# SeunghwanByun/SemanticSegmentation_Tensorflow

Hardware: AMD Instinct MI355X
Metric: train images/sec on KITTI 375×1242 2-class at 1/2/4/8 MI355X; mIoU parity (higher is better)
Workload: dtype bf16; 1 GPU; FCN (reference Network/model/FCN.py topology) train step: fwd + softmax-xent + bwd + TF1 Adam, 375x1242x3 zero-padded to 384x1248; global_batch=4, batch_per_gpu=4, image=375x1242 -> 384x1248, parallelism=dp1

## Files before the change

semanticsegmentation_tensorflow_amd/csrc/conv.hip:

```cpp
#include "common.h"
#include "igemm.h"
#include "halo.h"
#include <mutex>
#include <stdio.h>
#include <string.h>
#include <math.h>

using seg::NTParams;
using seg::TNParams;

static inline int round8(int c) { return (c + 7) & ~7; }

static int same_pads(int in, int k, int s, int d, int* out, int* pb, int* pa) {
    const int keff = k + (k - 1) * (d - 1);
    *out = (in + s - 1) / s;
    int total = (*out - 1) * s + keff - in;
    if (total < 0) total = 0;
    *pb = total / 2;
    *pa = total - total / 2;
    return 0;
}

static int valid_out(int in, int k, int s, int d) {
    const int keff = k + (k - 1) * (d - 1);
// ... 388 lines not shown
            macs = macs_conv;
            if (op == 1 && bwd_data_strided(d)) {
                if (!bwd_data_strided_ok(d)) return SEG_EINVAL;
                if (bwd_data_s2_runs(d, nullptr)) {
                    fam = "dgrad_s2"; bm = 256; bn = d->C >= 32 ? 32 : 16; sp = 1;
                    break;
                }
                NTParams p = bwd_data_strided_params(d);
                p.epi.n_valid = d->c_valid; p.epi.keep_prob = 1.f;
                fam = seg::nt_choice(p, d->dtype, d->stride_h * d->stride_w, p.M, &bm, &bn, &sp);
                break;
            }
            NTParams p = op == 0 ? conv_fwd_params(d) : conv_bwd_data_params(d);
            p.epi.keep_prob = 1.f;
            if (op == 0 && d->dil_w == d->dil_h && seg::smallc_fwd_ok(p, d->dtype, d->R, d->S, d->dil_h)) {
                fam = "conv_c8"; bm = 512; bn = d->K; sp = 1;
                break;
            }
            fam = seg::nt_choice(p, d->dtype, 1, p.M, &bm, &bn, &sp);
            break;
        }
        case 2: {
            TNParams p = conv_bwd_filter_params(d);
            seg::tn_info(p.M, p.N, p.P, d->dtype, &bm, &bn, &sp);
            fam = "igemm_tn";
            seg::WgradPlan wp;
            if (seg::smallc_wgrad_ok(p, d->dtype)) {
                fam = "wgrad_c8"; bm = 72; bn = p.N; sp = seg::smallc_wgrad_splits(p, seg::device_cus());
            } else if (g_tn_variant == 2 && seg::wgrad_plan(p, d->dtype, seg::device_cus(), &wp)) {
                fam = "wgrad_halo"; bm = 576; bn = wp.nt; sp = wp.splits;
            } else if (g_tn_variant == 2 && seg::tn3_ok(p, d->dtype)) {
                fam = "igemm_tn3"; bm = bn = 256; seg::tn3_info(p.M, p.N, p.P, seg::device_cus(), &sp);
            } else if (g_tn_variant == 2 && d->dtype != SEG_F32 && p.M >= 128) {
                fam = "igemm_tn2";
            }
            macs = macs_conv;
            break;
        }
        case 3: {
            macs = macs_t;
            if (const int kq = tconv_dense_kq(d)) {
                const int M = d->N * d->H * d->W, Nn = d->R * d->S * kq;
                NTParams g = dense_nt(M, Nn, d->C, nullptr, d->ldx, nullptr, nullptr, Nn);
                g.IH = d->H; g.IW = d->W; g.Ha = d->H; g.Wa = d->W; g.OH = d->H; g.OW = d->W;
                fam = seg::nt_choice(g, d->dtype, 1, g.M, &bm, &bn, &sp);
            } else {
                NTParams p = tconv_fwd_params(d);
                fam = seg::nt_choice(p, d->dtype, d->stride_h * d->stride_w, p.M, &bm, &bn, &sp);
            }
            break;
        }
        case 4: {
            macs = macs_t;
            if (const int kq = tconv_dense_kq(d)) {
                const int M = d->N * d->H * d->W, Kd = d->R * d->S * kq;
                NTParams g = dense_nt(M, d->C, Kd, nullptr, Kd, nullptr, nullptr, d->ldx);
                g.IH = d->H; g.IW = d->W; g.Ha = d->H; g.Wa = d->W; g.OH = d->H; g.OW = d->W;
                fam = seg::nt_choice(g, d->dtype, 1, g.M, &bm, &bn, &sp);
            } else {
                NTParams p = tconv_bwd_data_params(d);
                fam = seg::nt_choice(p, d->dtype, 1, p.M, &bm, &bn, &sp);
            }
            break;
        }
        case 5: {
            const int Mt = tconv_dense_kq(d) ? d->R * d->S * tconv_dense_kq(d) : d->R * d->S * d->K;
            seg::tn_info(Mt, d->C, d->N * d->H * d->W, d->dtype, &bm, &bn, &sp);
            fam = (g_tn_variant == 2 && d->dtype != SEG_F32 && Mt >= 128) ? "igemm_tn2" : "igemm_tn";
            if (g_tn_variant == 2 && seg::tn3_applies(Mt, d->C, d->dtype)) {
                fam = "igemm_tn3"; bm = bn = 256; seg::tn3_info(Mt, d->C, d->N * d->H * d->W, seg::device_cus(), &sp);
            }
            macs = macs_t;
            break;
        }
        case 6: {
            NTParams p;
            const int kind = bwd_data_bn_params(d, p);
            if (!kind) return SEG_EINVAL;
            macs = macs_conv;
            if (kind == 1 && seg::bn1x1s_ok(p, d->dtype)) { fam = "bn1x1_stream"; bm = 128; bn = 64; }
            else if (kind == 1) { fam = "igemm_nt2_bn"; bm = 256; bn = 64; }
            else { fam = "conv_res16c_bn"; bm = 256; bn = 64; }
            break;
        }
        case 7: {
            NTParams p = conv_fwd_params(d);
            macs = macs_conv;
            if (seg::s1x1_ok(p, d->dtype, 1)) {
                fam = "conv1x1_stream"; bm = 128; bn = 64;
            } else if (g_nt_variant == 2 && seg::nt2_pro_ok(p, d->dtype, 1)) {
                fam = "igemm_nt2_pro"; bm = 192; bn = p.N <= 64 ? 64 : 128;
            } else {
                fam = "igemm_nt_pro"; bm = 128; bn = p.N <= 64 ? 64 : 128;
            }
            break;
        }
        case 8: {
            TNParams p = conv_bwd_filter_params(d);
            macs = macs_conv;
            seg::tn_info(p.M, p.N, p.P, d->dtype, &bm, &bn, &sp);
            fam = (d->dtype != SEG_F32 && g_tn_variant == 2 && p.M == p.Cg) ? "igemm_tn2_pro" : "igemm_tn_pro";
            break;
        }
        default: return SEG_EINVAL;
    }
    if (name && len > 0) snprintf(name, len, "%s<%s,%d,%d>", fam, ty, bm, bn);
    if (splits) *splits = sp;
    if (flops) *flops = 2.0 * macs;
    return SEG_OK;
}

namespace {
struct Knob {
    const char* name;
    std::atomic<int> seg::KnobSet::*var;
    int lo, hi;
    int step;
    int only[8];
};

std::mutex g_knob_mu;

const Knob* find_knob(const char* name) {
    static const Knob knobs[] = {
        {"igemm_nt_variant", &seg::KnobSet::nt_variant, 1, 2, 1, {}},
        {"igemm_tn_variant", &seg::KnobSet::tn_variant, 1, 2, 1, {}},
        {"tn_nsplit", &seg::KnobSet::tn_nsplit, 0, 1, 1, {}},
        {"nt_nsplit", &seg::KnobSet::nt_nsplit, 0, 1, 1, {}},
        {"halo_duo", &seg::KnobSet::halo_duo, 0, 1, 1, {}},
        {"nt_halo", &seg::KnobSet::nt_halo, 0, 1, 1, {}},
        {"halo_wide", &seg::KnobSet::halo_wide, 0, 1, 1, {}},
        {"halo4", &seg::KnobSet::halo4, 0, 2, 1, {}},
        {"halo_min_splits", &seg::KnobSet::halo_min_splits, 1, 64, 1, {}},
        {"adam_tr_fused", &seg::KnobSet::adam_tr_fused, 0, 1, 1, {}},
        {"nt2_short", &seg::KnobSet::nt2_short, 0, 64, 1, {}},
        {"tn_fill", &seg::KnobSet::tn_fill, 1, 64, 1, {}},
        {"tn_split_cap", &seg::KnobSet::tn_split_cap, 1, 4096, 1, {}},
        {"tn_reduce_sl", &seg::KnobSet::tn_reduce_sl, 0, 0, 0, {1, 2, 4, 8, 16, 32, 64}},
        {"tn2_smallm", &seg::KnobSet::tn2_smallm, 0, 1, 1, {}},
        {"adam_blocks", &seg::KnobSet::adam_blocks, 0, 1 << 30, 1, {}},
        {"nt3_fill", &seg::KnobSet::nt3_fill, 0, 1, 1, {}},
        {"tn3_stagger_us", &seg::KnobSet::tn3_stagger_us, 0, 1000, 1, {}},
        {"s1x1", &seg::KnobSet::s1x1, 0, 1, 1, {}},
        {"tn3_half", &seg::KnobSet::tn3_half, 0, 7, 1, {}},
        {"tn3_mfast", &seg::KnobSet::tn3_mfast, 0, 1, 1, {}},
        {"tn3", &seg::KnobSet::tn3, 0, 1, 1, {}},
        {"nt3", &seg::KnobSet::nt3, 0, 1, 1, {}},
        {"wgrad_fill", &seg::KnobSet::wgrad_fill, 1, 800, 1, {}},
        {"wgrad_nt32", &seg::KnobSet::wgrad_nt32, 0, 1, 1, {}},
        {"wgrad_nbias", &seg::KnobSet::wgrad_nbias, 1, 4, 1, {}},
        {"wgrad_nt", &seg::KnobSet::wgrad_nt, 0, 0, 0, {64, 128}},
        {"wgrad_halo", &seg::KnobSet::wgrad_halo, 0, 1, 1, {}},
        {"wgrad_pxs", &seg::KnobSet::wgrad_pxs, 0, 1, 1, {}},
        {"smallc_tr", &seg::KnobSet::smallc_tr, 0, 1, 1, {}},
        {"res16c", &seg::KnobSet::res16c, 0, 1, 1, {}},
        {"res16", &seg::KnobSet::res16, 0, 1, 1, {}},
        {"res64", &seg::KnobSet::res64, 0, 1, 1, {}},
        {"res64_pp", &seg::KnobSet::res64_pp, 0, 2, 1, {}},
        {"res16_dma", &seg::KnobSet::res16_dma, 0, 1, 1, {}},
        {"res16c_bh", &seg::KnobSet::res16c_bh, 0, 0, 0, {4, 8}},
        {"bn1x1s", &seg::KnobSet::bn1x1s, 0, 1, 1, {}},
        {"s1x1_st", &seg::KnobSet::s1x1_st, 0, 2, 1, {}},
        {"res16c_st", &seg::KnobSet::res16c_st, 0, 1, 1, {}},
        {"dropout_flat", &seg::KnobSet::dropout_flat, 0, 1, 1, {}},
        {"smallc", &seg::KnobSet::smallc, 0, 1, 1, {}},
        {"smallk", &seg::KnobSet::smallk, 0, 1, 1, {}},
        {"wpad", &seg::KnobSet::wpad, 0, 256, 8, {}},
        {"dgrad_s2", &seg::KnobSet::dgrad_s2, 0, 1, 1, {}},
#ifdef SEG_DIAG
        {"tn3_abl", &seg::KnobSet::tn3_abl, 0, 3, 1, {}},
        {"smallk_abl", &seg::KnobSet::smallk_abl, 0, 3, 1, {}},
        {"tn3_adam_abl", &seg::KnobSet::tn3_adam_abl, 0, 31, 1, {}},
        {"wgrad_abl", &seg::KnobSet::wgrad_abl, 0, 3, 1, {}},
        {"nt2_ablate", &seg::KnobSet::nt2_ablate, 0, 19, 1, {}},
        {"res64_abl", &seg::KnobSet::res64_abl, 0, 5, 1, {}},
#endif
    };
    for (const Knob& k : knobs)
        if (!strcmp(name, k.name)) return &k;
    return nullptr;
}
}

namespace seg {
KnobSet& knobs() {
    constexpr int MAXDEV = 64;
    static KnobSet sets[MAXDEV];
    int d = 0;
    if (hipGetDevice(&d) != hipSuccess || d < 0 || d >= MAXDEV) d = 0;
    return sets[d];
}
}

extern "C" int seg_set_option(const char* name, int value) {
    const Knob* k = name ? find_knob(name) : nullptr;
    if (!k) return SEG_EINVAL;
    bool ok;
    if (k->step) {
        ok = value >= k->lo && value <= k->hi && (value - k->lo) % k->step == 0;
    } else {
        ok = false;
        for (int v : k->only) ok = ok || (v != 0 && v == value);
    }
    if (!ok) return SEG_EINVAL;
    std::lock_guard<std::mutex> lk(g_knob_mu);
    (seg::knobs().*(k->var)).store(value, std::memory_order_relaxed);
    return SEG_OK;
}

extern "C" int seg_get_option(const char* name, int* value) {
    const Knob* k = name ? find_knob(name) : nullptr;
    if (!k || !value) return SEG_EINVAL;
    *value = (seg::knobs().*(k->var)).load(std::memory_order_relaxed);
    return SEG_OK;
}

extern "C" int seg_conv2d_fwd(const seg_conv_desc* d, const void* x, const void* w, const seg_epilogue* epi,
                              void* y, void* ws, size_t ws_bytes, void* stream) {
    int st = check_desc(d);
    if (st) return st;
    if (!x || !w || !y) return SEG_EINVAL;
    NTParams p = conv_fwd_params(d);
    p.x = x; p.w = w; p.y = y;
    p.epi = make_epi(epi, d->k_valid, (long)d->OH * d->OW * (epi ? epi->ld_residual : 0));
    if (d->dil_w == d->dil_h && seg::smallc_fwd_ok(p, d->dtype, d->R, d->S, d->dil_h)) {
        seg::launch_smallc_fwd(p, d->dtype, (hipStream_t)stream);
        SEG_CHECK_LAUNCH();
        return SEG_OK;
    }
    return seg::launch_nt(p, d->dtype, 1, p.M, ws, ws_bytes, (hipStream_t)stream);
}

static bool fwd_relu_bits_params(const seg_conv_desc* d, const seg_epilogue* epi, int ld_bits, NTParams* out) {
    if (check_desc(d) || d->dil_w != d->dil_h || ld_bits < d->K / 8 || (d->K == 64 && ld_bits % 8)) return false;
    if (epi && epi->relu_mask) return false;
    NTParams p = conv_fwd_params(d);
    p.epi = make_epi(epi, d->k_valid, (long)d->OH * d->OW * (epi ? epi->ld_residual : 0));
    if (!seg::smallc_fwd_ok(p, d->dtype, d->R, d->S, d->dil_h)) return false;
    p.epi.ld_bits = ld_bits;
    *out = p;
    return true;
}

extern "C" int seg_conv2d_fwd_relu_bits_ok(const seg_conv_desc* d) {
    NTParams p;
    seg_epilogue e = {};
    e.relu = 1;
    e.keep_prob = 1.f;
    return d && fwd_relu_bits_params(d, &e, d->K / 8, &p) ? 1 : 0;
}

extern "C" int seg_conv2d_fwd_relu_bits(const seg_conv_desc* d, const void* x, const void* w, const seg_epilogue* epi,
                                        void* y, void* bits, int ld_bits, void* stream) {
    if (!d || !x || !w || !y || !bits) return SEG_EINVAL;
    if (d->K == 64 && ((uintptr_t)bits & 7)) return SEG_EALIGN;
    NTParams p;
    if (!fwd_relu_bits_params(d, epi, ld_bits, &p)) return SEG_EINVAL;
    p.x = x; p.w = w; p.y = y;
    p.epi.ybits = reinterpret_cast<unsigned char*>(bits);
    seg::launch_smallc_fwd(p, d->dtype, (hipStream_t)stream);
    SEG_CHECK_LAUNCH();
    return SEG_OK;
}

static NTParams fwd_hwio_params(const seg_conv_desc* d) {
    NTParams p = conv_fwd_params(d);
    p.bt = 1;
    p.w_col = d->K + g_wpad;
    p.w_tap = (long)d->C * (d->K + g_wpad);
    return p;
}

extern "C" int seg_conv2d_fwd_hwio_ok(const seg_conv_desc* d) {
    if (!d || check_desc(d) || (d->dtype != SEG_BF16 && d->dtype != SEG_F16)) return 0;
    return seg::nt_fwd_bt_ok(fwd_hwio_params(d), d->dtype) ? 1 : 0;
}

extern "C" int seg_conv2d_fwd_hwio(const seg_conv_desc* d, const void* x, const void* w_hwio, const seg_epilogue* epi,
                                   void* y, void* ws, size_t ws_bytes, void* stream) {
    int st = check_desc(d);
    if (st) return st;
    if (!x || !w_hwio || !y) return SEG_EINVAL;
    if (!seg_conv2d_fwd_hwio_ok(d)) return SEG_EINVAL;
    NTParams p = fwd_hwio_params(d);
    p.x = x; p.w = w_hwio; p.y = y;
    p.epi = make_epi(epi, d->k_valid, (long)d->OH * d->OW * (epi ? epi->ld_residual : 0));
    return seg::launch_nt(p, d->dtype, 1, p.M, ws, ws_bytes, (hipStream_t)stream);
}

static bool fwd_pool_params(const seg_conv_desc* d, const seg_epilogue* epi, NTParams* out) {
    if (check_desc(d) || (d->dtype != SEG_BF16 && d->dtype != SEG_F16)) return false;
    if ((d->OH & 1) || (d->OW & 1) || d->OH < 2 || d->OW < 2) return false;
    if (epi && (epi->scale || epi->shift || epi->residual || epi->relu_mask || (epi->keep_prob > 0.f && epi->keep_prob < 1.f)))
        return false;
    NTParams p = conv_fwd_params(d);
    p.epi = make_epi(epi, d->k_valid, 0);
    if (d->dil_w == d->dil_h && seg::smallc_fwd_ok(p, d->dtype, d->R, d->S, d->dil_h)) return false;
    if (!seg::nt_pool_ok(p, d->dtype)) return false;
    *out = p;
    return true;
}

extern "C" int seg_conv2d_fwd_pool_ok(const seg_conv_desc* d) {
    if (!d) return 0;
    NTParams p;
    seg_epilogue e = {};
// ... 635 lines not shown
```

semanticsegmentation_tensorflow_amd/csrc/knobs.h:

```cpp
#pragma once
#include <atomic>

namespace seg {

#define SEG_KNOBS(X) \
    X(wpad, 0) \
    X(adam_tr_fused, 0) \
    X(s1x1, 1) \
    X(bn1x1s, 1) \
    X(s1x1_st, 1) \
    X(dropout_flat, 1) \
    X(nt_halo, 1) \
    X(halo_wide, 1) \
    X(res64, 1) \
    X(res16, 1) \
    X(res64_pp, 1) \
    X(res64_abl, 0) \
    X(wgrad_pxs, 1) \
    X(smallc_tr, 1) \
    X(res16_dma, 1) \
    X(res16c_bh, 4) \
    X(res16c, 1) \
    X(halo_duo, 1) \
    X(halo_min_splits, 1) \
    X(res16c_st, 1) \
    X(halo4, 2) \
    X(nt_nsplit, 1) \
    X(tn_nsplit, 1) \
    X(nt_variant, 2) \
    X(nt3_fill, 1) \
    X(tn_variant, 2) \
    X(tn_fill, 2) \
    X(tn_split_cap, 256) \
    X(tn2_smallm, 0) \
    X(tn_reduce_sl, 16) \
    X(nt2_ablate, 0) \
    X(nt2_short, 8) \
    X(nt3, 1) \
    X(tn3, 1) \
    X(tn3_abl, 0) \
    X(tn3_mfast, 0) \
    X(tn3_half, 0) \
    X(tn3_stagger_us, 40) \
    X(tn3_adam_abl, 0) \
    X(adam_blocks, 0) \
    X(smallc, 1) \
    X(smallk, 1) \
    X(smallk_abl, 0) \
    X(wgrad_halo, 1) \
    X(wgrad_nt, 128) \
    X(wgrad_abl, 0) \
    X(wgrad_nt32, 1) \
    X(wgrad_fill, 88) \
    X(wgrad_nbias, 1) \
    X(dgrad_s2, 1)

struct KnobSet {
#define SEG_KNOB_MEMBER(n, d) std::atomic<int> n{d};
    SEG_KNOBS(SEG_KNOB_MEMBER)
#undef SEG_KNOB_MEMBER
};

KnobSet& knobs();

}

#define g_wpad (::seg::knobs().wpad.load(std::memory_order_relaxed))
#define g_adam_tr_fused (::seg::knobs().adam_tr_fused.load(std::memory_order_relaxed))
#define g_s1x1 (::seg::knobs().s1x1.load(std::memory_order_relaxed))
#define g_bn1x1s (::seg::knobs().bn1x1s.load(std::memory_order_relaxed))
#define g_s1x1_st (::seg::knobs().s1x1_st.load(std::memory_order_relaxed))
#define g_dropout_flat (::seg::knobs().dropout_flat.load(std::memory_order_relaxed))
#define g_nt_halo (::seg::knobs().nt_halo.load(std::memory_order_relaxed))
#define g_halo_wide (::seg::knobs().halo_wide.load(std::memory_order_relaxed))
#define g_res64 (::seg::knobs().res64.load(std::memory_order_relaxed))
#define g_res16 (::seg::knobs().res16.load(std::memory_order_relaxed))
#define g_res64_pp (::seg::knobs().res64_pp.load(std::memory_order_relaxed))
#define g_res64_abl (::seg::knobs().res64_abl.load(std::memory_order_relaxed))
#define g_wgrad_pxs (::seg::knobs().wgrad_pxs.load(std::memory_order_relaxed))
#define g_smallc_tr (::seg::knobs().smallc_tr.load(std::memory_order_relaxed))
#define g_res16_dma (::seg::knobs().res16_dma.load(std::memory_order_relaxed))
#define g_res16c_bh (::seg::knobs().res16c_bh.load(std::memory_order_relaxed))
#define g_res16c (::seg::knobs().res16c.load(std::memory_order_relaxed))
#define g_halo_duo (::seg::knobs().halo_duo.load(std::memory_order_relaxed))
#define g_halo_min_splits (::seg::knobs().halo_min_splits.load(std::memory_order_relaxed))
#define g_res16c_st (::seg::knobs().res16c_st.load(std::memory_order_relaxed))
#define g_halo4 (::seg::knobs().halo4.load(std::memory_order_relaxed))
#define g_nt_nsplit (::seg::knobs().nt_nsplit.load(std::memory_order_relaxed))
#define g_tn_nsplit (::seg::knobs().tn_nsplit.load(std::memory_order_relaxed))
#define g_nt_variant (::seg::knobs().nt_variant.load(std::memory_order_relaxed))
#define g_nt3_fill (::seg::knobs().nt3_fill.load(std::memory_order_relaxed))
#define g_tn_variant (::seg::knobs().tn_variant.load(std::memory_order_relaxed))
#define g_tn_fill (::seg::knobs().tn_fill.load(std::memory_order_relaxed))
#define g_tn_split_cap (::seg::knobs().tn_split_cap.load(std::memory_order_relaxed))
#define g_tn2_smallm (::seg::knobs().tn2_smallm.load(std::memory_order_relaxed))
#define g_tn_reduce_sl (::seg::knobs().tn_reduce_sl.load(std::memory_order_relaxed))
#define g_nt2_ablate (::seg::knobs().nt2_ablate.load(std::memory_order_relaxed))
#define g_nt2_short (::seg::knobs().nt2_short.load(std::memory_order_relaxed))
#define g_nt3 (::seg::knobs().nt3.load(std::memory_order_relaxed))
#define g_tn3 (::seg::knobs().tn3.load(std::memory_order_relaxed))
#define g_tn3_abl (::seg::knobs().tn3_abl.load(std::memory_order_relaxed))
#define g_tn3_mfast (::seg::knobs().tn3_mfast.load(std::memory_order_relaxed))
#define g_tn3_half (::seg::knobs().tn3_half.load(std::memory_order_relaxed))
#define g_tn3_stagger_us (::seg::knobs().tn3_stagger_us.load(std::memory_order_relaxed))
#define g_tn3_adam_abl (::seg::knobs().tn3_adam_abl.load(std::memory_order_relaxed))
#define g_adam_blocks (::seg::knobs().adam_blocks.load(std::memory_order_relaxed))
#define g_smallc (::seg::knobs().smallc.load(std::memory_order_relaxed))
#define g_smallk (::seg::knobs().smallk.load(std::memory_order_relaxed))
#define g_smallk_abl (::seg::knobs().smallk_abl.load(std::memory_order_relaxed))
#define g_wgrad_halo (::seg::knobs().wgrad_halo.load(std::memory_order_relaxed))
#define g_wgrad_nt (::seg::knobs().wgrad_nt.load(std::memory_order_relaxed))
#define g_wgrad_abl (::seg::knobs().wgrad_abl.load(std::memory_order_relaxed))
#define g_wgrad_nt32 (::seg::knobs().wgrad_nt32.load(std::memory_order_relaxed))
#define g_wgrad_fill (::seg::knobs().wgrad_fill.load(std::memory_order_relaxed))
#define g_wgrad_nbias (::seg::knobs().wgrad_nbias.load(std::memory_order_relaxed))
#define g_dgrad_s2 (::seg::knobs().dgrad_s2.load(std::memory_order_relaxed))
```

semanticsegmentation_tensorflow_amd/csrc/wgrad.hip:

```cpp
#include "common.h"
#include "igemm.h"
#include "ldsdma.h"

namespace seg {

static __device__ uint4 wg_zero_page[4];


struct WGGeom {
    int tiles_x, tiles_y, nimg, hwd, hrows;
    int nct, nnt, splits, tps, ptiles;
    int nbias;
};

template <int ROWB>
__device__ __forceinline__ int wg_swz(int row) {
    if constexpr (ROWB >= 256) return ((row & 3) << 1) | (((row >> 3) & 1) << 3);
    else if constexpr (ROWB == 64) return 0;
    else return (((row >> 1) & 1) << 1) | (((row >> 3) & 1) << 2);
}

template <int NT, int NST, int HI, int ABL = 0, typename T = bf16, bool PXS = false>
__global__ __launch_bounds__(512) void wgrad_halo(TNParams p, WGGeom g) {
    constexpr int BW = 16;
    using V8 = vec8_t<T>;
    constexpr int NW = 8, BH = 128 / BW;
    constexpr int NF = PXS ? NT / 16 : NT / 32;
    static_assert(!PXS || NT == 64, "pixel-split waves hold all 64 columns");
    constexpr int DROWB = NT * 2;
    constexpr int D_RPI = 1024 / DROWB;
    constexpr int D_INS = 128 / D_RPI / NW;
    constexpr int D_CPR = DROWB / 16;
    constexpr int HBUF = HI * NW * 1024;
    constexpr int DBUF = 128 * DROWB;
    constexpr int STAGE = HBUF + DBUF;
    static_assert(BW == 16 || BW == 32, "8-pixel fragment groups must stay in one tile row");
    __shared__ __attribute__((aligned(16))) char smem[NST * STAGE];

    const int nout = g.nct * g.nnt;
    const int wg = xcd_remap2(blockIdx.x, gridDim.x);
    const int split = wg / nout, ot = wg - (wg / nout) * nout;
    if (split >= g.splits) return;
    const int ct = ot / g.nnt, nt = ot - (ot / g.nnt) * g.nnt;
    const int c0 = ct * 64, n0 = nt * NT;
    const int t_begin = split * g.tps, t_end = min(g.ptiles, t_begin + g.tps);

    const int tid = threadIdx.x, lane = tid & 63;
    const int w = __builtin_amdgcn_readfirstlane(tid >> 6);
    const int cf = w & 3;
    const int nh = PXS ? 0 : w >> 2;
    const int ph = PXS ? w >> 2 : 0;
    const T* __restrict__ X = reinterpret_cast<const T*>(p.x);
    const T* __restrict__ Dy = reinterpret_cast<const T*>(p.b);
    const void* zero = (const void*)wg_zero_page;

    const int lr = lane >> 3;
    const int hc = (lane & 7) ^ ((((lr >> 1) & 1) << 1) | ((w & 1) << 2));
    int h_hy[HI], h_hx[HI];
#pragma unroll
    for (int h = 0; h < HI; ++h) {
        const int hr = (h * NW + w) * 8 + lr;
        h_hy[h] = hr < g.hrows ? hr / g.hwd : -(1 << 20);
        h_hx[h] = hr < g.hrows ? hr - (hr / g.hwd) * g.hwd : 0;
    }
    const int h_n = g.hrows > w * 8 ? min(HI, (g.hrows - w * 8 + NW * 8 - 1) / (NW * 8)) : 0;
    const int dr = lane / D_CPR, dpc = lane % D_CPR;
    int dc;
    if constexpr (DROWB >= 256) dc = dpc ^ (((dr & 3) << 1) | (((w >> 1) & 1) << 3));
    else if constexpr (DROWB == 64) dc = dpc;
    else dc = dpc ^ ((((dr >> 1) & 1) << 1) | ((w & 1) << 2));
    const bool d_nok = n0 + dc * 8 < p.N;

    const unsigned lds0 = (unsigned)(uintptr_t)(SEG_LDS char*)smem;
    auto stage_tile = [&](int t, int buf) {
        const int tpi = g.tiles_x * g.tiles_y;
        const int img = t / tpi;
        const int rem = t - img * tpi;
        const int ty = rem / g.tiles_x, tx = rem - (rem / g.tiles_x) * g.tiles_x;
        const int oy0 = ty * BH, ox0 = tx * BW;
        const long xb = (long)img * p.x_img + c0 + hc * 8;
        const unsigned sb = lds0 + buf * STAGE;
#pragma unroll
        for (int h = 0; h < HI; ++h) {
            if (h < h_n) {
                const int ih = oy0 + p.ioh + h_hy[h], iw = ox0 + p.iow + h_hx[h];
                const bool ok = (unsigned)ih < (unsigned)p.IH && (unsigned)iw < (unsigned)p.IW;
                const void* src = ok ? (const void*)(X + xb + ((long)ih * p.IW + iw) * p.ldx) : zero;
                glds16(src, sb + (h * NW + w) * 1024);
            }
        }
#pragma unroll
        for (int i = 0; i < D_INS; ++i) {
            const int r = (i * NW + w) * D_RPI + dr;
            const int oy = oy0 + r / BW, ox = ox0 + r % BW;
            const bool ok = d_nok && oy < p.Ha && ox < p.Wa;
            const void* src =
                ok ? (const void*)(Dy + (((long)img * p.Ha + oy) * p.Wa + ox) * p.ldb + n0 + dc * 8) : zero;
            glds16(src, sb + HBUF + (i * NW + w) * 1024);
        }
    };

    f32x4 acc[9][NF];
#pragma unroll
    for (int i = 0; i < 9; ++i)
#pragma unroll
        for (int j = 0; j < NF; ++j) acc[i][j] = f32x4{0.f, 0.f, 0.f, 0.f};
    const bool do_bias = p.dbias != nullptr && ct < g.nbias && cf < NF;
    float dsum[NF];
#pragma unroll
    for (int j = 0; j < NF; ++j) dsum[j] = 0.f;

    const int fg = lane >> 4, tq = (lane & 15) >> 2, tpp = lane & 3;
    typedef short s16x8 __attribute__((ext_vector_type(8)));
    int tapoff[9];
#pragma unroll
    for (int r = 0; r < 3; ++r)
#pragma unroll
        for (int s = 0; s < 3; ++s) tapoff[r * 3 + s] = r * p.tsh * g.hwd + s * p.tsw;

    unsigned a_pk[9], b_pk[NF];
    {
        const int kk = 8 * fg + tq;
        const int py = kk / BW, px = kk - (kk / BW) * BW;
        const int achk = cf * 2 + (tpp >> 1);
#pragma unroll
        for (int t = 0; t < 9; ++t) {
            const int r1 = py * g.hwd + px + tapoff[t];
            const unsigned lo = r1 * 128 + 16 * (achk ^ wg_swz<128>(r1)) + 8 * (tpp & 1);
            const unsigned hi = (r1 + 4) * 128 + 16 * (achk ^ wg_swz<128>(r1 + 4)) + 8 * (tpp & 1);
            a_pk[t] = lo | (hi << 16);
        }
        const int d1 = wg_swz<DROWB>(kk), d2 = wg_swz<DROWB>(kk + 4);
#pragma unroll
        for (int ni = 0; ni < NF; ++ni) {
            const int chk = ((nh * (NT / 2) + ni * 16) >> 3) + (tpp >> 1);
            const unsigned lo = kk * DROWB + 16 * ((chk & ~15) | ((chk & 15) ^ d1)) + 8 * (tpp & 1);
            const unsigned hi = (kk + 4) * DROWB + 16 * ((chk & ~15) | ((chk & 15) ^ d2)) + 8 * (tpp & 1);
            b_pk[ni] = lo | (hi << 16);
        }
    }
    const int per_tile = h_n + D_INS;
    for (int i = 0; i < NST - 1; ++i)
        if (t_begin + i < t_end) stage_tile(t_begin + i, i);
    int buf = 0;
    for (int t = t_begin; t < t_end; ++t) {
        const int younger = min(NST - 2, t_end - 1 - t);
        const int allow = younger * per_tile;
        if (allow <= 0) wait_vmcnt<0>();
        else if (allow <= 2) wait_vmcnt<2>();
        else if (allow <= 3) wait_vmcnt<3>();
        else if (allow <= 4) wait_vmcnt<4>();
        else if (allow <= 5) wait_vmcnt<5>();
        else if (allow <= 6) wait_vmcnt<6>();
        else if (allow <= 7) wait_vmcnt<7>();
        else if (allow <= 8) wait_vmcnt<8>();
        else if (allow <= 9) wait_vmcnt<9>();
        else if (allow <= 10) wait_vmcnt<10>();
        else if (allow <= 11) wait_vmcnt<11>();
        else wait_vmcnt<12>();
        lds_barrier();
        if (ABL != 1 && t + NST - 1 < t_end) stage_tile(t + NST - 1, buf == 0 ? NST - 1 : buf - 1);
        auto read_b = [&](int ss, V8* bo) {
            if constexpr (ABL == 3) {
#pragma unroll
                for (int ni = 0; ni < NF; ++ni) {
                    s16x8 v = {(short)ss, (short)ni, 1, 2, 3, 4, 5, (short)lane};
                    bo[ni] = __builtin_bit_cast(V8, v);
                }
                return;
            }
#pragma unroll
            for (int ni = 0; ni < NF; ++ni) {
                SEG_LDS char* dbs = (SEG_LDS char*)smem + buf * STAGE + HBUF + ss * 32 * DROWB;
                const s16x4 lo = __builtin_amdgcn_ds_read_tr16_b64_v4i16((SEG_LDS s16x4*)(dbs + (b_pk[ni] & 0xffffu)));
                const s16x4 hi = __builtin_amdgcn_ds_read_tr16_b64_v4i16((SEG_LDS s16x4*)(dbs + (b_pk[ni] >> 16)));
                s16x8 v = {lo[0], lo[1], lo[2], lo[3], hi[0], hi[1], hi[2], hi[3]};
                bo[ni] = __builtin_bit_cast(V8, v);
                if (do_bias && ni == cf && ss % g.nbias == ct) {
#pragma unroll
                    for (int e = 0; e < 8; ++e)
                        dsum[ni] += bits16_to_f32<T>((unsigned short)v[e]);
                }
            }
        };
        auto read_a = [&](int ss, int tap) {
            if constexpr (ABL == 3) {
                s16x8 v = {(short)ss, (short)tap, 1, 2, 3, 4, 5, (short)lane};
                return __builtin_bit_cast(V8, v);
            }
            SEG_LDS char* hb = (SEG_LDS char*)smem + buf * STAGE + ss * (32 / BW) * g.hwd * 128;
            const s16x4 lo = __builtin_amdgcn_ds_read_tr16_b64_v4i16((SEG_LDS s16x4*)(hb + (a_pk[tap] & 0xffffu)));
            const s16x4 hi = __builtin_amdgcn_ds_read_tr16_b64_v4i16((SEG_LDS s16x4*)(hb + (a_pk[tap] >> 16)));
            s16x8 v = {lo[0], lo[1], lo[2], lo[3], hi[0], hi[1], hi[2], hi[3]};
            return __builtin_bit_cast(V8, v);
        };
        const int ss0 = 2 * ph;
        V8 b0[NF], b1[NF];
        read_b(ss0, b0);
        V8 a_cur = read_a(ss0, 0);
        auto substep = [&](int ss, V8* bc, V8* bn, bool more) {
#pragma unroll
            for (int tap = 0; tap < 9; ++tap) {
                V8 a_nxt = a_cur;
                if (tap < 8) a_nxt = read_a(ss, tap + 1);
                else if (more) a_nxt = read_a(ss + 1, 0);
                if (tap == 4 && more) read_b(ss + 1, bn);
#pragma unroll
                for (int ni = 0; ni < NF; ++ni) {
                    if constexpr (ABL == 2) asm volatile("" ::"v"(a_cur), "v"(bc[ni]));
                    else acc[tap][ni] = mfma_v8<T>(a_cur, bc[ni], acc[tap][ni]);
                }
                a_cur = a_nxt;
            }
        };
        if constexpr (PXS) {
            substep(ss0, b0, b1, true);
            substep(ss0 + 1, b1, b0, false);
        } else {
#pragma unroll 1
            for (int ss = 0; ss < 4; ss += 2) {
                substep(ss, b0, b1, true);
                substep(ss + 1, b1, b0, ss + 2 < 4);
            }
        }
        buf = buf == NST - 1 ? 0 : buf + 1;
    }
    const int fr = lane & 15;
    const int slab = PXS ? 2 * split + ph : split;
    if (do_bias) {
#pragma unroll
        for (int ni = 0; ni < NF; ++ni) {
            dsum[ni] += __shfl_xor(dsum[ni], 16);
            dsum[ni] += __shfl_xor(dsum[ni], 32);
        }
        if (fg == 0) {
#pragma unroll
            for (int ni = 0; ni < NF; ++ni) {
                if (ni != cf) continue;
                const int n = n0 + nh * (NT / 2) + ni * 16 + fr;
                if (p.partial) {
                    if (n < p.N) p.partial[((long)slab * p.Mp + p.M + ct) * p.N + n] = dsum[ni];
                } else if (n < p.n_valid) {
                    p.dbias[n] = dsum[ni];
                }
            }
        }
    }
#pragma unroll
    for (int tap = 0; tap < 9; ++tap)
#pragma unroll
        for (int j = 0; j < 4; ++j) {
            const int c = c0 + cf * 16 + fg * 4 + j;
            const int m = tap * p.Cg + c;
            if (p.partial) {
                float* prow = p.partial + ((long)slab * p.Mp + m) * p.N;
#pragma unroll
                for (int ni = 0; ni < NF; ++ni) {
                    const int n = n0 + nh * (NT / 2) + ni * 16 + fr;
                    if (n < p.N) prow[n] = acc[tap][ni][j];
                }
            } else if (c < p.c_valid) {
                float* orow = p.out + (long)tap * p.o_tap + (long)c * p.o_c;
#pragma unroll
                for (int ni = 0; ni < NF; ++ni) {
                    const int n = n0 + nh * (NT / 2) + ni * 16 + fr;
                    if (n < p.n_valid) orow[(long)n * p.o_n] = acc[tap][ni][j];
                }
            }
        }
}

bool wgrad_plan(const TNParams& p, int dtype, int cus, WgradPlan* wp) {
    if (!g_wgrad_halo || (dtype != SEG_BF16 && dtype != SEG_F16)) return false;
    if (p.ish != 1 || p.isw != 1 || p.taps_w != 3 || p.Cg % 64 != 0 || p.M != 9 * p.Cg) return false;
    if (p.tsh <= 0 || p.tsw <= 0 || p.N % 8 != 0 || p.ldb % 8 != 0 || p.ldx % 8 != 0) return false;
    if (p.Ha <= 0 || p.Wa <= 0 || p.P % (p.Ha * p.Wa) != 0) return false;
    const int nimg = p.P / (p.Ha * p.Wa);
    const int bw = 16, bh = 128 / bw;
    const int hwd = (bw + 2 * p.tsw + 7) & ~7;
    const int hrows = hwd * (bh + 2 * p.tsh);
    if (hrows > 5 * 64) return false;
    wp->bw = bw;
    wp->g[0] = (p.Wa + bw - 1) / bw; wp->g[1] = (p.Ha + bh - 1) / bh; wp->g[3] = hwd; wp->g[4] = hrows;
    wp->nt = (g_wgrad_nt == 128 && p.N > 64 && wp->g[4] <= 4 * 64) ? 128 : 64;
    if (g_wgrad_nt32 && p.N <= 32) wp->nt = 32;
    wp->g[2] = nimg;
    const int nct = p.Cg / 64, nnt = (p.N + wp->nt - 1) / wp->nt;
    const int nout = nct * nnt;
    const int ptiles = nimg * wp->g[0] * wp->g[1];
    const int tcus = std::max(1, cus * g_wgrad_fill / 100);
    int splits = std::max(1, std::min(ptiles, one_round_splits(nout, tcus, ptiles)));
    const int tps = (ptiles + splits - 1) / splits;
    splits = (ptiles + tps - 1) / tps;
    wp->g[5] = nct; wp->g[6] = nnt; wp->g[7] = splits; wp->g[8] = tps; wp->g[9] = ptiles;
    wp->splits = splits;
    wp->pxs = wp->nt == 64 && g_wgrad_pxs && splits > 1;
    wp->slabs = splits * (wp->pxs ? 2 : 1);
    wp->nbias = splits > 1 ? std::max(1, std::min(nct, g_wgrad_nbias)) : 1;
    wp->blocks = (long)nout * splits;
    return true;
}

size_t wgrad_workspace(const WgradPlan& wp, const TNParams& p) {
    return wp.slabs > 1 ? (size_t)wp.slabs * (p.M + wp.nbias) * p.N * sizeof(float) : 0;
}

void launch_wgrad(TNParams& p, const WgradPlan& wp, hipStream_t s, int dtype) {
    WGGeom g;
    g.tiles_x = wp.g[0]; g.tiles_y = wp.g[1]; g.nimg = wp.g[2]; g.hwd = wp.g[3]; g.hrows = wp.g[4];
    g.nct = wp.g[5]; g.nnt = wp.g[6]; g.splits = wp.g[7]; g.tps = wp.g[8]; g.ptiles = wp.g[9];
    g.nbias = wp.nbias;
    const dim3 grid((unsigned)wp.blocks), block(512);
    const bool small = g.hrows <= 4 * 64;
#ifdef SEG_DIAG
    if (g_wgrad_abl && wp.nt == 128 && dtype == SEG_BF16) {
        if (g_wgrad_abl == 1) hipLaunchKernelGGL((wgrad_halo<128, 2, 4, 1>), grid, block, 0, s, p, g);
        if (g_wgrad_abl == 2) hipLaunchKernelGGL((wgrad_halo<128, 2, 4, 2>), grid, block, 0, s, p, g);
        if (g_wgrad_abl == 3) hipLaunchKernelGGL((wgrad_halo<128, 2, 4, 3>), grid, block, 0, s, p, g);
        return;
    }
#endif
    if (wp.pxs) {
        if (dtype == SEG_F16) {
            if (small) hipLaunchKernelGGL((wgrad_halo<64, 3, 4, 0, f16, true>), grid, block, 0, s, p, g);
            else hipLaunchKernelGGL((wgrad_halo<64, 2, 5, 0, f16, true>), grid, block, 0, s, p, g);
        } else {
            if (small) hipLaunchKernelGGL((wgrad_halo<64, 3, 4, 0, bf16, true>), grid, block, 0, s, p, g);
            else hipLaunchKernelGGL((wgrad_halo<64, 2, 5, 0, bf16, true>), grid, block, 0, s, p, g);
        }
        return;
    }
    if (dtype == SEG_F16) {
        if (wp.nt == 128) hipLaunchKernelGGL((wgrad_halo<128, 2, 4, 0, f16>), grid, block, 0, s, p, g);
        else if (wp.nt == 32 && small) hipLaunchKernelGGL((wgrad_halo<32, 3, 4, 0, f16>), grid, block, 0, s, p, g);
        else if (wp.nt == 32) hipLaunchKernelGGL((wgrad_halo<32, 2, 5, 0, f16>), grid, block, 0, s, p, g);
        else if (small) hipLaunchKernelGGL((wgrad_halo<64, 3, 4, 0, f16>), grid, block, 0, s, p, g);
        else hipLaunchKernelGGL((wgrad_halo<64, 2, 5, 0, f16>), grid, block, 0, s, p, g);
        return;
    }
    if (wp.nt == 128) hipLaunchKernelGGL((wgrad_halo<128, 2, 4>), grid, block, 0, s, p, g);
    else if (wp.nt == 32 && small) hipLaunchKernelGGL((wgrad_halo<32, 3, 4>), grid, block, 0, s, p, g);
    else if (wp.nt == 32) hipLaunchKernelGGL((wgrad_halo<32, 2, 5>), grid, block, 0, s, p, g);
    else if (small) hipLaunchKernelGGL((wgrad_halo<64, 3, 4>), grid, block, 0, s, p, g);
    else hipLaunchKernelGGL((wgrad_halo<64, 2, 5>), grid, block, 0, s, p, g);
}

}
```

Measured before the change: 609.9 images/s.

## Interleave wgrad halo tile staging loads between MFMA groups

Adds an SB variant of the wgrad_halo kernel. It precomputes buffer resource descriptors and per-piece offsets, then issues the next tile's global-to-LDS loads one piece at a time after every second MFMA tap, rather than in a single burst before compute. Tile and image indices are advanced incrementally instead of being recomputed with divisions. The goal is to hide load issue and address arithmetic behind matrix math. In exchange it uses more registers, and it is gated by a 31-bit range check on buffer sizes.

```diff
diff --git a/semanticsegmentation_tensorflow_amd/csrc/conv.hip b/semanticsegmentation_tensorflow_amd/csrc/conv.hip
--- a/semanticsegmentation_tensorflow_amd/csrc/conv.hip
+++ b/semanticsegmentation_tensorflow_amd/csrc/conv.hip
@@ -564,6 +564,7 @@
         {"wgrad_nt", &seg::KnobSet::wgrad_nt, 0, 0, 0, {64, 128}},
         {"wgrad_halo", &seg::KnobSet::wgrad_halo, 0, 1, 1, {}},
         {"wgrad_pxs", &seg::KnobSet::wgrad_pxs, 0, 1, 1, {}},
+        {"wgrad_stage", &seg::KnobSet::wgrad_stage, 0, 1, 1, {}},
         {"smallc_tr", &seg::KnobSet::smallc_tr, 0, 1, 1, {}},
         {"res16c", &seg::KnobSet::res16c, 0, 1, 1, {}},
         {"res16", &seg::KnobSet::res16, 0, 1, 1, {}},
diff --git a/semanticsegmentation_tensorflow_amd/csrc/knobs.h b/semanticsegmentation_tensorflow_amd/csrc/knobs.h
--- a/semanticsegmentation_tensorflow_amd/csrc/knobs.h
+++ b/semanticsegmentation_tensorflow_amd/csrc/knobs.h
@@ -53,6 +53,7 @@
     X(wgrad_nt32, 1) \
     X(wgrad_fill, 88) \
     X(wgrad_nbias, 1) \
+    X(wgrad_stage, 1) \
     X(dgrad_s2, 1)
 
 struct KnobSet {
@@ -114,4 +115,5 @@
 #define g_wgrad_nt32 (::seg::knobs().wgrad_nt32.load(std::memory_order_relaxed))
 #define g_wgrad_fill (::seg::knobs().wgrad_fill.load(std::memory_order_relaxed))
 #define g_wgrad_nbias (::seg::knobs().wgrad_nbias.load(std::memory_order_relaxed))
+#define g_wgrad_stage (::seg::knobs().wgrad_stage.load(std::memory_order_relaxed))
 #define g_dgrad_s2 (::seg::knobs().dgrad_s2.load(std::memory_order_relaxed))
diff --git a/semanticsegmentation_tensorflow_amd/csrc/wgrad.hip b/semanticsegmentation_tensorflow_amd/csrc/wgrad.hip
--- a/semanticsegmentation_tensorflow_amd/csrc/wgrad.hip
+++ b/semanticsegmentation_tensorflow_amd/csrc/wgrad.hip
@@ -20,7 +20,7 @@
     else return (((row >> 1) & 1) << 1) | (((row >> 3) & 1) << 2);
 }
 
-template <int NT, int NST, int HI, int ABL = 0, typename T = bf16, bool PXS = false>
+template <int NT, int NST, int HI, int ABL = 0, typename T = bf16, bool PXS = false, bool SB = false>
 __global__ __launch_bounds__(512) void wgrad_halo(TNParams p, WGGeom g) {
     constexpr int BW = 16;
     using V8 = vec8_t<T>;
@@ -72,6 +72,84 @@
     const bool d_nok = n0 + dc * 8 < p.N;
 
     const unsigned lds0 = (unsigned)(uintptr_t)(SEG_LDS char*)smem;
+
+    constexpr unsigned OOB = 0x80000000u;
+    constexpr int NPIECE = HI + D_INS;
+    const unsigned hv0 = (unsigned)((lr * p.ldx + hc * 8) * 2);
+    const unsigned dv0 = d_nok ? (unsigned)((dr * p.ldb + dc * 8) * 2) : OOB;
+    int p_hy[HI], p_hx[HI];
+    unsigned p_off[HI];
+#pragma unroll
+    for (int h = 0; h < HI; ++h) {
+        const int hr0 = (h * NW + w) * 8;
+        p_hy[h] = hr0 / g.hwd;
+        p_hx[h] = hr0 - p_hy[h] * g.hwd;
+        p_off[h] = (unsigned)((p_hy[h] * p.IW + p_hx[h]) * p.ldx * 2);
+    }
+    int s_tx = 0, s_ty = 0;
+    unsigned s_xoff = 0, s_doff = 0;
+    const T* s_xb = X;
+    const T* s_db = Dy;
+    seg_i32x4 rs_x = {0, 0, 0, 0x00020000}, rs_d = {0, 0, 0, 0x00020000};
+    auto s_set_img = [&]() {
+        const uint64_t xa = (uint64_t)(uintptr_t)s_xb, da = (uint64_t)(uintptr_t)s_db;
+        rs_x.x = (int)(unsigned)xa; rs_x.y = (int)((xa >> 32) & 0xffffu);
+        rs_d.x = (int)(unsigned)da; rs_d.y = (int)((da >> 32) & 0xffffu);
+    };
+    auto s_set_tile = [&]() {
+        s_xoff = (unsigned)((((s_ty * BH) * p.IW + s_tx * BW) * p.ldx + c0) * 2);
+        s_doff = (unsigned)((((s_ty * BH) * p.Wa + s_tx * BW) * p.ldb + n0) * 2);
+    };
+    auto s_advance = [&]() {
+        if (++s_tx == g.tiles_x) {
+            s_tx = 0;
+            if (++s_ty == g.tiles_y) {
+                s_ty = 0;
+                s_xb += p.x_img;
+                s_db += (long)p.Ha * p.Wa * p.ldb;
+                s_set_img();
+            }
+        }
+        s_set_tile();
+    };
+    if constexpr (SB) {
+        const int tpi = g.tiles_x * g.tiles_y;
+        const int img = t_begin / tpi;
+        const int rem = t_begin - img * tpi;
+        s_ty = rem / g.tiles_x;
+        s_tx = rem - s_ty * g.tiles_x;
+        const int shift = (p.ioh * p.IW + p.iow) * p.ldx;
+        s_xb = X + (long)img * p.x_img + shift;
+        s_db = Dy + (long)img * p.Ha * p.Wa * p.ldb;
+        rs_x.z = (p.IH * p.IW * p.ldx - shift) * 2;
+        rs_d.z = p.Ha * p.Wa * p.ldb * 2;
+        s_set_img();
+        s_set_tile();
+    }
+    auto s_piece = [&](const int K, unsigned sb) __attribute__((always_inline)) {
+        if (K < HI) {
+            if (K < h_n) {
+                const bool rok = (unsigned)(s_ty * BH + p.ioh + p_hy[K]) < (unsigned)p.IH;
+                const bool cok = (unsigned)(s_tx * BW + p.iow + p_hx[K] + lr) < (unsigned)p.IW;
+                bglds16(rs_x, rok && cok ? hv0 : OOB, rok ? s_xoff + p_off[K] : 0u, sb + (K * NW + w) * 1024);
+            }
+        } else if (K < NPIECE) {
+            const int I = K - HI;
+            const int rr = (I * NW + w) * D_RPI;
+            const int oyo = rr / BW, oxo = rr % BW;
+            const bool rok = s_ty * BH + oyo < p.Ha;
+            const bool cok = s_tx * BW + oxo + dr < p.Wa;
+            bglds16(rs_d, rok && cok ? dv0 : OOB, rok ? s_doff + (unsigned)((oyo * p.Wa + oxo) * p.ldb * 2) : 0u,
+                    sb + HBUF + (I * NW + w) * 1024);
+        }
+    };
+    auto s_burst = [&](unsigned sb) {
+#pragma unroll
+        for (int k = 0; k < NPIECE; ++k) s_piece(k, sb);
+        s_advance();
+    };
+    static_assert(NPIECE <= 9, "one piece after every second MFMA group of two substeps");
+
     auto stage_tile = [&](int t, int buf) {
         const int tpi = g.tiles_x * g.tiles_y;
         const int img = t / tpi;
@@ -141,7 +219,10 @@
     }
     const int per_tile = h_n + D_INS;
     for (int i = 0; i < NST - 1; ++i)
-        if (t_begin + i < t_end) stage_tile(t_begin + i, i);
+        if (t_begin + i < t_end) {
+            if constexpr (SB) s_burst(lds0 + i * STAGE);
+            else stage_tile(t_begin + i, i);
+        }
     int buf = 0;
     for (int t = t_begin; t < t_end; ++t) {
         const int younger = min(NST - 2, t_end - 1 - t);
@@ -159,7 +240,11 @@
         else if (allow <= 11) wait_vmcnt<11>();
         else wait_vmcnt<12>();
         lds_barrier();
-        if (ABL != 1 && t + NST - 1 < t_end) stage_tile(t + NST - 1, buf == 0 ? NST - 1 : buf - 1);
+        const bool st_on = ABL != 1 && t + NST - 1 < t_end;
+        const unsigned st_sb = lds0 + (buf == 0 ? NST - 1 : buf - 1) * STAGE;
+        if constexpr (!SB) {
+            if (st_on) stage_tile(t + NST - 1, buf == 0 ? NST - 1 : buf - 1);
+        }
         auto read_b = [&](int ss, V8* bo) {
             if constexpr (ABL == 3) {
 #pragma unroll
@@ -198,7 +283,8 @@
         V8 b0[NF], b1[NF];
         read_b(ss0, b0);
         V8 a_cur = read_a(ss0, 0);
-        auto substep = [&](int ss, V8* bc, V8* bn, bool more) {
+        auto substep = [&](int ss, V8* bc, V8* bn, bool more, bool st, auto sec_tag) __attribute__((always_inline)) {
+            constexpr int G0 = decltype(sec_tag)::value ? 9 : 0;
 #pragma unroll
             for (int tap = 0; tap < 9; ++tap) {
                 V8 a_nxt = a_cur;
@@ -211,16 +297,28 @@
                     else acc[tap][ni] = mfma_v8<T>(a_cur, bc[ni], acc[tap][ni]);
                 }
                 a_cur = a_nxt;
+                if constexpr (SB) {
+                    if ((G0 + tap) % 2 == 0 && (G0 + tap) / 2 < NPIECE) {
+                        if (st) s_piece((G0 + tap) / 2, st_sb);
+                    }
+                }
             }
         };
         if constexpr (PXS) {
-            substep(ss0, b0, b1, true);
-            substep(ss0 + 1, b1, b0, false);
+            substep(ss0, b0, b1, true, st_on, std::false_type{});
+            substep(ss0 + 1, b1, b0, false, st_on, std::true_type{});
+            if constexpr (SB) {
+                if (st_on) s_advance();
+            }
         } else {
 #pragma unroll 1
             for (int ss = 0; ss < 4; ss += 2) {
-                substep(ss, b0, b1, true);
-                substep(ss + 1, b1, b0, ss + 2 < 4);
+                const bool st = st_on && ss == 0;
+                substep(ss, b0, b1, true, st, std::false_type{});
+                substep(ss + 1, b1, b0, ss + 2 < 4, st, std::true_type{});
+                if constexpr (SB) {
+                    if (st) s_advance();
+                }
             }
         }
         buf = buf == NST - 1 ? 0 : buf + 1;
@@ -305,44 +403,58 @@
     return wp.slabs > 1 ? (size_t)wp.slabs * (p.M + wp.nbias) * p.N * sizeof(float) : 0;
 }
 
+static bool wgrad_stage_ok(const TNParams& p) {
+    const long shift = ((long)p.ioh * p.IW + p.iow) * p.ldx;
+    const long xb = ((long)(p.IH + 32) * p.IW * p.ldx + std::labs(shift)) * 2;
+    const long db = (long)(p.Ha + 32) * p.Wa * p.ldb * 2;
+    return (long)p.IH * p.IW * p.ldx - shift > 0 && xb < (1L << 31) && db < (1L << 31);
+}
+
+template <int NT, int NST, int HI, int ABL, typename T, bool PXS>
+static void wgrad_launch1(bool sb, dim3 grid, hipStream_t s, const TNParams& p, const WGGeom& g) {
+    if (sb) hipLaunchKernelGGL((wgrad_halo<NT, NST, HI, ABL, T, PXS, true>), grid, dim3(512), 0, s, p, g);
+    else hipLaunchKernelGGL((wgrad_halo<NT, NST, HI, ABL, T, PXS, false>), grid, dim3(512), 0, s, p, g);
+}
+
 void launch_wgrad(TNParams& p, const WgradPlan& wp, hipStream_t s, int dtype) {
     WGGeom g;
     g.tiles_x = wp.g[0]; g.tiles_y = wp.g[1]; g.nimg = wp.g[2]; g.hwd = wp.g[3]; g.hrows = wp.g[4];
     g.nct = wp.g[5]; g.nnt = wp.g[6]; g.splits = wp.g[7]; g.tps = wp.g[8]; g.ptiles = wp.g[9];
     g.nbias = wp.nbias;
-    const dim3 grid((unsigned)wp.blocks), block(512);
+    const dim3 grid((unsigned)wp.blocks);
     const bool small = g.hrows <= 4 * 64;
+    const bool sb = g_wgrad_stage && wgrad_stage_ok(p);
 #ifdef SEG_DIAG
     if (g_wgrad_abl && wp.nt == 128 && dtype == SEG_BF16) {
-        if (g_wgrad_abl == 1) hipLaunchKernelGGL((wgrad_halo<128, 2, 4, 1>), grid, block, 0, s, p, g);
-        if (g_wgrad_abl == 2) hipLaunchKernelGGL((wgrad_halo<128, 2, 4, 2>), grid, block, 0, s, p, g);
-        if (g_wgrad_abl == 3) hipLaunchKernelGGL((wgrad_halo<128, 2, 4, 3>), grid, block, 0, s, p, g);
+        if (g_wgrad_abl == 1) wgrad_launch1<128, 2, 4, 1, bf16, false>(sb, grid, s, p, g);
+        if (g_wgrad_abl == 2) wgrad_launch1<128, 2, 4, 2, bf16, false>(sb, grid, s, p, g);
+        if (g_wgrad_abl == 3) wgrad_launch1<128, 2, 4, 3, bf16, false>(sb, grid, s, p, g);
         return;
     }
 #endif
     if (wp.pxs) {
         if (dtype == SEG_F16) {
-            if (small) hipLaunchKernelGGL((wgrad_halo<64, 3, 4, 0, f16, true>), grid, block, 0, s, p, g);
-            else hipLaunchKernelGGL((wgrad_halo<64, 2, 5, 0, f16, true>), grid, block, 0, s, p, g);
+            if (small) wgrad_launch1<64, 3, 4, 0, f16, true>(sb, grid, s, p, g);
+            else wgrad_launch1<64, 2, 5, 0, f16, true>(sb, grid, s, p, g);
         } else {
-            if (small) hipLaunchKernelGGL((wgrad_halo<64, 3, 4, 0, bf16, true>), grid, block, 0, s, p, g);
-            else hipLaunchKernelGGL((wgrad_halo<64, 2, 5, 0, bf16, true>), grid, block, 0, s, p, g);
+            if (small) wgrad_launch1<64, 3, 4, 0, bf16, true>(sb, grid, s, p, g);
+            else wgrad_launch1<64, 2, 5, 0, bf16, true>(sb, grid, s, p, g);
         }
         return;
     }
     if (dtype == SEG_F16) {
-        if (wp.nt == 128) hipLaunchKernelGGL((wgrad_halo<128, 2, 4, 0, f16>), grid, block, 0, s, p, g);
-        else if (wp.nt == 32 && small) hipLaunchKernelGGL((wgrad_halo<32, 3, 4, 0, f16>), grid, block, 0, s, p, g);
-        else if (wp.nt == 32) hipLaunchKernelGGL((wgrad_halo<32, 2, 5, 0, f16>), grid, block, 0, s, p, g);
-        else if (small) hipLaunchKernelGGL((wgrad_halo<64, 3, 4, 0, f16>), grid, block, 0, s, p, g);
-        else hipLaunchKernelGGL((wgrad_halo<64, 2, 5, 0, f16>), grid, block, 0, s, p, g);
+        if (wp.nt == 128) wgrad_launch1<128, 2, 4, 0, f16, false>(sb, grid, s, p, g);
+        else if (wp.nt == 32 && small) wgrad_launch1<32, 3, 4, 0, f16, false>(sb, grid, s, p, g);
+        else if (wp.nt == 32) wgrad_launch1<32, 2, 5, 0, f16, false>(sb, grid, s, p, g);
+        else if (small) wgrad_launch1<64, 3, 4, 0, f16, false>(sb, grid, s, p, g);
+        else wgrad_launch1<64, 2, 5, 0, f16, false>(sb, grid, s, p, g);
         return;
     }
-    if (wp.nt == 128) hipLaunchKernelGGL((wgrad_halo<128, 2, 4>), grid, block, 0, s, p, g);
-    else if (wp.nt == 32 && small) hipLaunchKernelGGL((wgrad_halo<32, 3, 4>), grid, block, 0, s, p, g);
-    else if (wp.nt == 32) hipLaunchKernelGGL((wgrad_halo<32, 2, 5>), grid, block, 0, s, p, g);
-    else if (small) hipLaunchKernelGGL((wgrad_halo<64, 3, 4>), grid, block, 0, s, p, g);
-    else hipLaunchKernelGGL((wgrad_halo<64, 2, 5>), grid, block, 0, s, p, g);
-}
-
-}
+    if (wp.nt == 128) wgrad_launch1<128, 2, 4, 0, bf16, false>(sb, grid, s, p, g);
+    else if (wp.nt == 32 && small) wgrad_launch1<32, 3, 4, 0, bf16, false>(sb, grid, s, p, g);
+    else if (wp.nt == 32) wgrad_launch1<32, 2, 5, 0, bf16, false>(sb, grid, s, p, g);
+    else if (small) wgrad_launch1<64, 3, 4, 0, bf16, false>(sb, grid, s, p, g);
+    else wgrad_launch1<64, 2, 5, 0, bf16, false>(sb, grid, s, p, g);
+}
+
+}
```

After: 615.5 images/s, median of 6. No clear change (+0.9%).
